# xdsopl/dwt

Hardware: AMD Instinct MI355X
Metric: Mpixels/s lossless encode+decode round-trip (higher is better)
Workload: dtype int32; 1 GPU; 4096x4096x1 8-bit synthetic smooth+noise frames, lossless, 128 frames per GPU per step (BASELINE.json configs[1] geometry); frames_per_gpu=128, parallelism=1 GPU

## Files before the change

dwt_amd/csrc/pack.hip:

```cpp
#include "hilbert_dev.h"

#include <stdlib.h>
#include <string.h>

namespace {

constexpr int TILE = 1024;
constexpr int NCUM = 32;
constexpr int MAX_PLANES = 16;
constexpr int MAX_SEGS = 3 * 16 * MAX_PLANES;
constexpr int SUB = 64;
constexpr int CHUNK = SUB * 64;
constexpr int GROUP = 64;

constexpr unsigned T_RUN = 0x0fffu, T_ESC = 0x0fffu, T_BREAK = 1u << 13, T_VOID = 1u << 14, T_NOSIGN = 1u << 15;

struct PackGeom {
	int levels, C, W, H;
	long total;
	const int *pyr;
	const short *fine16;
	unsigned lv16;
	unsigned sq_levels;
	int pixels[DWTX_MAX_LEVELS + 1];
// ... 1713 lines not shown

__global__ __launch_bounds__(1024) void k_chain_image(Work w)
{
	const int img = blockIdx.x;
	if (!w.slow[img])
		return;
	const ImgInfo &I = w.info[img];
	const long nchunks = ((long)I.T + CHUNK - 1) / CHUNK;
	const long ngroups = (nchunks + GROUP - 1) / GROUP;
	unsigned char *gentry = w.group_entry + img * w.NGS;
	if (threadIdx.x == 0) {
		int o = I.order0;
		for (long gq = 0; gq < ngroups; ++gq) {
			gentry[gq] = (unsigned char)o;
			o = w.glut[(img * w.NGS + gq) * 32 + o];
		}
	}
	__syncthreads();
	__threadfence_block();
	const unsigned char *lut = w.lut + img * w.NCS * 32;
	unsigned char *centry = w.chunk_entry + img * w.NCS;
	for (long gq = threadIdx.x; gq < ngroups; gq += 1024) {
		int o = gentry[gq];
		for (long c = gq * GROUP; c < min((gq + 1) * GROUP, nchunks); ++c) {
			centry[c] = (unsigned char)o;
			o = lut[c * 32 + o];
		}
	}
}

__device__ __forceinline__ void gorder_exact_body(const Work &w, unsigned *rows, long chunk, int img)
{
	const int lane = threadIdx.x & 63;
	const ImgInfo &I = w.info[img];
	const long T = I.T;
	const long nchunks = (T + CHUNK - 1) / CHUNK;
	if (chunk >= nchunks)
		return;
	const unsigned short *tok16 = w.tok16 + img * w.TS;
	const unsigned *big = w.tok_big + img * w.TS;
	wave_sync();
	stage_tokens(rows, tok16, chunk * CHUNK, T, lane);
	wave_sync();
	const long S = chunk * 64 + lane;
	const int o = w.sublut[((img * w.NCS + chunk) * 64 + lane) * 32 + w.chunk_entry[img * w.NCS + chunk]];
	const bool produces = S * SUB < T;
	unsigned tokbits = 0;
	unsigned long long rawbits = 0;
	walk_bits(rows + lane * WROW, big, S * SUB, o, 16, produces, w.brk_tok + (long)img * MAX_SEGS, w.seg_refs + (long)img * MAX_SEGS, I.K,
		tokbits, rawbits);
	unsigned long long total;
	const unsigned long long pre = wave_excl_scan64(produces ? tokbits + rawbits : 0ull, total);
	if (produces) {
		w.lane_bits[img * w.NCS * 64 + S] = pre;
		w.grp_ord[img * w.NCS * 64 + S] = (unsigned char)o;
	}
	if (lane == 0)
		w.chunk_bits[img * w.NCS + chunk] = total;
}

__global__ __launch_bounds__(256) void k_gorder_exact(Work w)
{
	__shared__ WalkLds lds[4];
	const int img = blockIdx.y;
	if (!w.slow[img])
		return;
	const long nvb = (w.NCS + 3) / 4;
	for (long vb = blockIdx.x; vb < nvb; vb += gridDim.x)
		gorder_exact_body(w, lds[threadIdx.x >> 6].tok, vb * 4 + (threadIdx.x >> 6), img);
}

constexpr int EWIN = 768;

struct EmitLds {
	unsigned tok[64 * HROW];
	unsigned win[EWIN];
};

__global__ __launch_bounds__(256) __attribute__((amdgpu_waves_per_eu(5))) void k_emit(Work w, unsigned *out, long out_words)
{
	__shared__ EmitLds lds[4];
	const int lane = threadIdx.x & 63, wv = threadIdx.x >> 6;
	const long wave = (long)blockIdx.x * 4 + wv;
	const int img = blockIdx.y;
	const ImgInfo &I = w.info[img];
	const long T = I.T;
	const long ngroups = (T + SUB - 1) / SUB;
	if (wave * 64 >= ngroups)
		return;
	const unsigned short *tok16 = w.tok16 + img * w.TS;
	const unsigned *big = w.tok_big + img * w.TS;
	const unsigned *srefs = w.seg_refs + (long)img * MAX_SEGS;
	const unsigned *btok = w.brk_tok + (long)img * MAX_SEGS;
	unsigned *rows = lds[wv].tok, *win = lds[wv].win;
	for (int i = lane; i < EWIN; i += 64)
		win[i] = 0u;
	const long S = wave * 64 + lane;
	const bool live = S < ngroups;
	const int per = w.slow[img] ? 64 : FSUBS;
	unsigned long long pos = 0;
	int o = 0;
	if (live) {
		pos = w.chunk_base[img * w.NCS + S / per] + w.lane_bits[img * w.NCS * 64 + S];
		o = w.grp_ord[img * w.NCS * 64 + S];
	}
	const long wbase = (long)(__shfl(pos, 0) >> 5);
	unsigned *dst = out + img * out_words;
	wave_sync();
	auto put_word = [&](long wi, unsigned v) {
		if (!v)
			return;
		const unsigned long rel = (unsigned long)(wi - wbase);
		if (rel < (unsigned long)EWIN)
			__hip_atomic_fetch_or((__attribute__((address_space(3))) unsigned *)win + rel, v, __ATOMIC_RELAXED, __HIP_MEMORY_SCOPE_WORKGROUP);
		else if (wi < out_words)
			atomicOr(dst + wi, v);
	};
	long widx = (long)(pos >> 5);
	int fill = (int)(pos & 31);
	unsigned long long acc = 0;
	auto append = [&](unsigned c, int n) {
		acc |= (unsigned long long)c << fill;
		fill += n;
		if (fill >= 32) {
			put_word(widx, (unsigned)acc);
			++widx;
			acc >>= 32;
			fill -= 32;
		}
	};
	const unsigned *my = rows + lane * HROW;
	const long tb = S * SUB;
	auto slow_token = [&](unsigned tk, long t) {
		if (!(tk & T_VOID)) {
			const unsigned v = token_run(tk, big, t);
			const int top = vli_top(o, v);
			const int z = top - o;
			const unsigned rem = v + (1u << o) - (1u << top);
			unsigned long long code = (1ull << z) | ((unsigned long long)rem << (z + 1));
			int len = z + 1 + top;
			if (!(tk & T_NOSIGN)) {
				code |= (unsigned long long)((tk >> 12) & 1u) << len;
				++len;
			}
			o = vli_next(top);
			append((unsigned)code, len < 32 ? len : 32);
			if (len > 32)
				append((unsigned)(code >> 32), len - 32);
		}
		if (tk & T_BREAK) {
			put_word(widx, (unsigned)acc);
			acc = 0;
			const long k = find_break_seg(btok, I.K, (unsigned)t);
			const unsigned long long at = ((unsigned long long)widx << 5) + (unsigned)fill;
			w.seg_rawoff[(long)img * MAX_SEGS + k] = at;
			const unsigned long long next = at + srefs[k];
			widx = (long)(next >> 5);
			fill = (int)(next & 31);
		}
	};
	auto code16 = [&](unsigned tk, unsigned &code, int &len) {
		const unsigned s = (tk & T_RUN) + (1u << o);
		const int top = 31 - __builtin_clz(s);
		const int z = top - o;
		const unsigned rem = s & bfm_mask((unsigned)top);
		const int l = z + 1 + top;
		code = (rem << (z + 1)) | (1u << z) | (((tk >> 12) & 1u) << l);
		len = l + ((tk & T_NOSIGN) ? 0 : 1);
		o = (int)__builtin_elementwise_sub_sat((unsigned)top, 2u);
	};
	HalfTokens staged = load_tokens_half(tok16, wave * CHUNK, T, lane, 0);
	for (int half = 0; half < 2; ++half) {
		if (half)
			wave_sync();
		deposit_tokens_half(rows, staged, lane);
		if (!half)
			staged = load_tokens_half(tok16, wave * CHUNK, T, lane, 1);
		wave_sync();
		if (!live)
			continue;
#pragma unroll 2
		for (int q8 = 0; q8 < 8; ++q8) {
			const int q = half * 8 + q8;
			const uint2 x2 = *reinterpret_cast<const uint2 *>(my + 2 * q8);
			const unsigned xs[2] = { x2.x, x2.y };
#pragma unroll
			for (int h = 0; h < 2; ++h) {
				const unsigned x = xs[h];
				if ((x & ((0x0f80u | T_BREAK | T_VOID) * 0x00010001u)) != 0u || o > 7) {
					slow_token(x & 0xffffu, tb + 4 * q + 2 * h);
					slow_token(x >> 16, tb + 4 * q + 2 * h + 1);
				} else {
					unsigned c0, c1;
					int l0, l1;
					code16(x & 0xffffu, c0, l0);
					code16(x >> 16, c1, l1);
					acc |= (unsigned long long)(c0 | (c1 << l0)) << fill;
					fill += l0 + l1;
					if (fill >= 32) {
						put_word(widx, (unsigned)acc);
						++widx;
						acc >>= 32;
						fill -= 32;
					}
				}
			}
		}
	}
	if (live)
		put_word(widx, (unsigned)acc);
	const long nlive = ngroups - wave * 64 < 64 ? ngroups - wave * 64 : 64;
	const long endw = __shfl(widx, (int)nlive - 1);
	wave_sync();
	for (int i = lane; i < EWIN; i += 64) {
		const long wi = wbase + i;
		if (wi - i + (i & ~63) > endw)
			break;
		if (wi > endw || wi >= out_words)
			continue;
		const unsigned v = win[i];
		if (wi > wbase && wi < endw)
			dst[wi] = v;
		else if (v)
			atomicOr(dst + wi, v);
	}
}

__global__ __launch_bounds__(1024) void k_bitscan(Work w, long capacity)
{
	__shared__ unsigned long long wsum[16];
	__shared__ unsigned long long carry;
	const int img = blockIdx.x;
	ImgInfo &I = w.info[img];
	const long nsub = ((long)I.T + SUB - 1) / SUB;
	const long nchunks = w.slow[img] ? ((long)I.T + CHUNK - 1) / CHUNK : (nsub + FSUBS - 1) / FSUBS;
	const unsigned long long *cb = w.chunk_bits + img * w.NCS;
	unsigned long long *base = w.chunk_base + img * w.NCS;
	const int lane = threadIdx.x & 63, wv = threadIdx.x >> 6;
	if (threadIdx.x == 0)
		carry = I.hdr_bits;
	__syncthreads();
	for (long b0 = 0; b0 < nchunks; b0 += 1024) {
		const long i = b0 + threadIdx.x;
		const unsigned long long v = i < nchunks ? cb[i] : 0ull;
		unsigned long long inc = v;
		for (int o = 1; o < 64; o <<= 1) {
			const unsigned long long t = __shfl_up(inc, o);
			if (lane >= o)
				inc += t;
		}
		if (lane == 63)
			wsum[wv] = inc;
		__syncthreads();
		unsigned long long woff = 0, all = 0;
		for (int k = 0; k < 16; ++k) {
			const unsigned long long s = wsum[k];
			woff += k < wv ? s : 0ull;
			all += s;
		}
		const unsigned long long c = carry;
		if (i < nchunks)
			base[i] = c + woff + inc - v;
		__syncthreads();
		if (threadIdx.x == 0)
			carry = c + all;
		__syncthreads();
	}
	if (threadIdx.x == 0) {
		const unsigned long long bits = carry;
		w.stream_bits[img] = bits;
		unsigned long long bytes = (bits + 7) >> 3;
		I.total_bits = bits;
		if (capacity > 0 && bytes > (unsigned long long)capacity) {
			bytes = (unsigned long long)capacity;
			if (bits >= 8ull * ((unsigned long long)capacity + 1))
				I.total_bits = bytes * 8;
		}
		I.nbytes = bytes;
		I.pad = w.slow[img];
	}
}

__global__ __launch_bounds__(256) void k_clear_stream(Work w, unsigned *out, long out_words)
{
	const int img = blockIdx.y;
	const long first = ((long)w.info[img].hdr_bits + 31) >> 5;
	long last = (long)((w.stream_bits[img] + 31) >> 5) + 4;
	last = last < out_words ? last : out_words;
	unsigned *base = out + img * out_words;
	const bool vec = ((uintptr_t)base & 15) == 0;
	for (long i = ((first & ~3l) >> 2) + (long)blockIdx.x * blockDim.x + threadIdx.x; i * 4 < last; i += (long)gridDim.x * blockDim.x) {
		unsigned *dst = base + i * 4;
		if (vec && i * 4 >= first && i * 4 + 4 <= last) {
			*reinterpret_cast<uint4 *>(dst) = make_uint4(0u, 0u, 0u, 0u);
		} else {
			for (int k = 0; k < 4; ++k)
				if (i * 4 + k >= first && i * 4 + k < last)
					dst[k] = 0u;
		}
	}
}

constexpr int REF_WIN = 2048;

__global__ __launch_bounds__(256) void k_refcopy(Work w, unsigned *out, long out_words)
{
	const int img = blockIdx.y;
	const int K = w.info[img].K;
	const int *eb = w.seg_ebase + (long)img * (MAX_SEGS + 1);
	const unsigned *refscum = w.ent_refscum + img * (w.ES + 1), *refw = w.ent_refw + img * (w.ES + 1);
	const unsigned short *erefs = w.ent_refs + img * w.ES;
	const unsigned *stage = w.stage + img * w.SW;
	unsigned *dst = out + img * out_words;
	__shared__ unsigned win[REF_WIN + 2];
	__shared__ unsigned wfirst[MAX_SEGS + 1];
	__shared__ unsigned wsum[4];
	{
		unsigned mine[3], sum = 0;
#pragma unroll
		for (int u = 0; u < 3; ++u) {
			const int k = 3 * (int)threadIdx.x + u;
			unsigned nwin = 0;
			if (k < K) {
				const unsigned n = w.seg_refs[(long)img * MAX_SEGS + k];
				if (n) {
					const unsigned long long D = w.seg_rawoff[(long)img * MAX_SEGS + k];
					const unsigned long words = (unsigned long)(((D + n - 1) >> 5) - (D >> 5) + 1);
					nwin = (unsigned)((words + REF_WIN - 1) / REF_WIN);
				}
			}
			mine[u] = nwin;
			sum += nwin;
		}
		unsigned total;
		const unsigned pre = block_excl_scan(sum, wsum, total);
		unsigned run = pre;
#pragma unroll
		for (int u = 0; u < 3; ++u) {
			const int k = 3 * (int)threadIdx.x + u;
			wfirst[k] = run;
			run += mine[u];
		}
		if (threadIdx.x == blockDim.x - 1)
			wfirst[MAX_SEGS] = run;
		__syncthreads();
	}
	const unsigned nwin_all = wfirst[K < MAX_SEGS ? K : MAX_SEGS];
	for (unsigned vw = blockIdx.x; vw < nwin_all; vw += gridDim.x) {
		int lo = 0, hi = K - 1;
		while (lo < hi) {
			const int mid = (lo + hi + 1) >> 1;
			if (wfirst[mid] <= vw)
				lo = mid;
			else
				hi = mid - 1;
		}
		const int k = lo;
		const unsigned wi = vw - wfirst[k];
		const unsigned n = w.seg_refs[(long)img * MAX_SEGS + k];
		const unsigned long long D = w.seg_rawoff[(long)img * MAX_SEGS + k];
		const long d0 = (long)(D >> 5), dl = (long)((D + n - 1) >> 5);
		const long ws = d0 + (long)wi * REF_WIN;
		const int nwords = (int)(dl - ws + 1 < REF_WIN ? dl - ws + 1 : REF_WIN);
		const long long x0 = ((long long)ws << 5) - (long long)D, x1 = x0 + 32ll * nwords;
		for (int i = threadIdx.x; i < nwords + 2; i += blockDim.x)
			win[i] = 0u;
		__syncthreads();
		const int e0 = eb[k], e1 = eb[k + 1];
		const unsigned cbase = refscum[e0];
		int a = e0, b = e1 - 1;
		while (a < b) {
			const int mid = (a + b + 1) >> 1;
			if ((long long)(refscum[mid] - cbase) <= (x0 > 0 ? x0 : 0))
				a = mid;
			else
				b = mid - 1;
		}
		for (int ea = a; ea < e1; ea += blockDim.x) {
			const int e = ea + (int)threadIdx.x;
			const long long c = e < e1 ? (long long)(refscum[e] - cbase) : x1;
			if (__syncthreads_and(c >= x1))
				break;
			const unsigned r = e < e1 ? erefs[e] : 0u;
			if (!r || c >= x1)
				continue;
			const unsigned *src = stage + refw[e];
			const int nsrc = (int)((r + 31u) >> 5);
			for (int jw = 0; jw < nsrc; ++jw) {
				const long long o = c + 32ll * jw - x0;
				if (o <= -32 || o >= 32ll * nwords)
					continue;
				const unsigned v = src[jw];
				const long long ob = o + 32;
				const int idx = (int)(ob >> 5), sh = (int)(ob & 31);
				if (v) {
					atomicOr(&win[idx], v << sh);
					if (sh && idx + 1 < nwords + 2)
						atomicOr(&win[idx + 1], v >> (32 - sh));
				}
			}
		}
		__syncthreads();
		for (int i = threadIdx.x; i < nwords; i += blockDim.x) {
			const long wd = ws + i;
			if (wd >= out_words)
				continue;
			const unsigned v = win[1 + i];
			if (wd == d0 || wd == dl) {
				if (v)
					atomicOr(dst + wd, v);
			} else {
				dst[wd] = v;
			}
		}
		__syncthreads();
	}
}

constexpr int IDX_THREADS = 832;
static_assert(IDX_THREADS > MAX_SEGS && IDX_THREADS % 64 == 0, "one lane per segment and one for the header");

__global__ __launch_bounds__(IDX_THREADS) void k_index(PackGeom g, Work w, dwtx_index *index)
{
	__shared__ unsigned long long wsum[IDX_THREADS / 64];
	__shared__ unsigned nxt[IDX_THREADS];
	__shared__ unsigned btok[MAX_SEGS], srefs[MAX_SEGS];
	const int img = blockIdx.x;
	const ImgInfo &I = w.info[img];
	dwtx_index &X = index[img];
	const int K = I.K;
	const bool whole = I.nbytes >= (w.stream_bits[img] + 7) >> 3;
	if (K <= 0 || I.pmax <= 0 || I.error || I.cut || !whole) {
		if (threadIdx.x == 0) {
			X.magic = DWTX_INDEX_MAGIC;
			X.W = g.W;
			X.H = g.H;
			X.C = g.C;
			X.nsegs = 0;
			X.reserved = 0;
			X.stream_bits = 0ull;
		}
		return;
	}
	const int k = threadIdx.x, lane = threadIdx.x & 63, wv = wave_in_block();
	const int *sd = w.seg_desc + (long)img * MAX_SEGS;
	int num = 0;
	if (k < K) {
		int c, l, p;
		seg_unpack(sd[k], c, l, p);
		num = g.pixels[l + 1] - g.pixels[l];
	}
	const long T = I.T;
	const unsigned short *tok16 = w.tok16 + img * w.TS;
	const unsigned *big = w.tok_big + img * w.TS;
	if (k < K) {
		btok[k] = w.brk_tok[(long)img * MAX_SEGS + k];
		srefs[k] = w.seg_refs[(long)img * MAX_SEGS + k];
	}
	long t0 = T - 1;
	if (k < K) {
		t0 = w.ent_tokbase[img * (w.ES + 1) + w.seg_ebase[(long)img * (MAX_SEGS + 1) + k]];
		nxt[k] = (tok16[t0] & T_VOID) ? (unsigned)(T - 1) : (unsigned)t0;
	} else {
		nxt[k] = (unsigned)(T - 1);
	}
	unsigned long long wtot;
	unsigned long long sym_base = wave_excl_scan64(((unsigned long long)num + 31ull) & ~31ull, wtot);
	if (lane == 0)
		wsum[wv] = wtot;
	__syncthreads();
	for (int i = 0; i < wv; ++i)
		sym_base += wsum[i];
	for (int d = 1; d < IDX_THREADS; d <<= 1) {
		const unsigned a = nxt[k], b = k + d < IDX_THREADS ? nxt[k + d] : a;
		__syncthreads();
		nxt[k] = a < b ? a : b;
		__syncthreads();
	}
	if (k > K)
		return;
	const unsigned j = k < K ? w.seg_run[(long)img * MAX_SEGS + k] : 0u;
	const long tt = j ? (long)nxt[k] : t0;
	const long S = tt / SUB;
	const int per = w.slow[img] ? 64 : FSUBS;
	unsigned long long pos = w.chunk_base[img * w.NCS + S / per] + w.lane_bits[img * w.NCS * 64 + S];
	int o = w.grp_ord[img * w.NCS * 64 + S];
	uint4 grp[8];
#pragma unroll
	for (int q = 0; q < 8; ++q)
		grp[q] = *reinterpret_cast<const uint4 *>(tok16 + S * SUB + 8 * q);
	const int before = (int)(tt - S * SUB);
	int kb = (int)find_break_seg(btok, K, (unsigned)(S * SUB));
#pragma unroll
	for (int q = 0; q < 32; ++q) {
		const uint4 x4 = grp[q >> 2];
		const unsigned x = (q & 3) == 0 ? x4.x : (q & 3) == 1 ? x4.y : (q & 3) == 2 ? x4.z : x4.w;
#pragma unroll
		for (int h = 0; h < 2; ++h) {
			const unsigned tk = h ? x >> 16 : x & 0xffffu;
			const long t = S * SUB + 2 * q + h;
			if (2 * q + h < before) {
				if (!(tk & T_VOID)) {
					const int top = vli_top(o, token_run(tk, big, t));
					pos += (unsigned)(2 * top - o + 1) + ((tk & T_NOSIGN) ? 0u : 1u);
					o = vli_next(top);
				}
				if (tk & T_BREAK)
					pos += srefs[kb++];
			}
		}
	}
	const unsigned v = token_run(tok16[tt], big, tt);
	if (k < K ? j != 0u : v != 0u) {
		const int top = vli_top(o, v);
		pos += (unsigned)(2 * top - o + 1);
		o = vli_next(top);
	}
	if (k < K) {
		dwtx_seg_index &e = X.seg[k];
		e.bit = pos;
		e.sym_base = sym_base;
		e.n1 = (unsigned)num - srefs[k];
		e.cnt = j ? v - j + 1u : 0u;
		e.desc = (unsigned)sd[k];
		e.order = (unsigned)o;
	} else {
		X.magic = DWTX_INDEX_MAGIC;
		X.W = g.W;
		X.H = g.H;
		X.C = g.C;
		X.nsegs = K;
		X.reserved = 0;
		X.stream_bits = pos;
	}
}

}


extern "C" int dwtx_encode_planes(dwtx_ctx *ctx, const int32_t *lin, int W, int H, int C, int n, long capacity,
	uint8_t *out, size_t out_stride, dwtx_stream_info *dev_info)
{
	return dwtx_encode_planes_ex(ctx, lin, nullptr, 0u, 0u, W, H, C, n, capacity, out, out_stride, dev_info, dwtx_p16{ nullptr, 0u },
		ctx ? ctx->enc_index : nullptr);
}

static int pack_geometry(dwtx_ctx *ctx, int W, int H, int C, int n, PackGeom &g, Work &w, dwtx_tiles &tiles)
{
	const int rc = dwtx_fill_geom(ctx, W, H, C, g, tiles);
	if (rc)
		return rc;
	g.tile_cnt = tiles.cnt;
	memset(&w, 0, sizeof(w));
	w.NT = tiles.NT;
	w.NTP = (tiles.NT + 3) / 4 * 4;
	const size_t nplanes = (size_t)n * C;
	const bool ok = carve(ctx, SLOT_PK_CUM, [&](Carve &c) {
		c.take(w.cum, nplanes * w.NT * NCUM);
		c.take(w.tile_mx, nplanes * w.NTP);
	});
	return ok ? DWTX_OK : DWTX_ERR_NOMEM;
}

int dwtx_hist_begin(dwtx_ctx *ctx, int W, int H, int C, int n, dwtx_hist_sink *sink)
{
	if (!ctx || !sink || (C != 1 && C != 3) || n < 1 || !dwtx_count_ok((long)n * C, DWTX_MAX_PLANES_PER_CALL, "planes"))
		return DWTX_ERR_ARG;
	DWTX_ENTER(ctx);
	DWTX_CHECK_DIMS(W, H);
	PackGeom g;
	Work w;
	dwtx_tiles tiles;
	const int rc = pack_geometry(ctx, W, H, C, n, g, w, tiles);
	if (rc)
		return rc;
	hipLaunchKernelGGL(k_hist_init, dim3(dwtx_cdiv(w.NT * (NCUM / 2), 256), n * C), dim3(256), 0, ctx->stream, g, w);
	DWTX_LAUNCH_CHECK();
	sink->cum32 = reinterpret_cast<unsigned *>(w.cum);
	sink->tile_mx = w.tile_mx;
	sink->NT = w.NT;
	sink->NTP = w.NTP;
	sink->tiles = tiles;
	return DWTX_OK;
}

#ifdef DWTX_DEBUG_HOOKS
extern "C" int dwtx_debug_hist_copy(dwtx_ctx *ctx, int W, int H, int C, int n, unsigned *host_cum32, unsigned *host_mx, int *NT, int *NTP, int *tile_first)
{
	PackGeom g;
	Work w;
	dwtx_tiles tiles;
	const int rc = pack_geometry(ctx, W, H, C, n, g, w, tiles);
	if (rc)
		return rc;
	*NT = w.NT;
	*NTP = w.NTP;
	for (int l = 0; l <= g.levels; ++l)
		tile_first[l] = tiles.tile_first[l];
	if (host_cum32) {
		DWTX_HIP(hipMemcpyAsync(host_cum32, w.cum, sizeof(unsigned) * 16 * (size_t)n * C * w.NT, hipMemcpyDeviceToHost, ctx->stream));
		DWTX_HIP(hipMemcpyAsync(host_mx, w.tile_mx, sizeof(unsigned) * (size_t)n * C * w.NTP, hipMemcpyDeviceToHost, ctx->stream));
		DWTX_HIP(hipStreamSynchronize(ctx->stream));
	}
	return DWTX_OK;
}
#endif

int dwtx_encode_planes_ex(dwtx_ctx *ctx, const int32_t *lin, const int32_t *pyr, unsigned sq_levels, unsigned hist_levels, int W, int H, int C,
	int n, long capacity, uint8_t *out, size_t out_stride, dwtx_stream_info *dev_info, dwtx_p16 p16, dwtx_index *dev_index)
{
	if (!ctx || !lin || !out || !dev_info || (C != 1 && C != 3) || n < 1 || (out_stride & 3) || out_stride < 8 ||
		!dwtx_count_ok((long)n * C, DWTX_MAX_PLANES_PER_CALL, "planes"))
		return DWTX_ERR_ARG;
	DWTX_ENTER(ctx);
	DWTX_CHECK_DIMS(W, H);
	if (sq_levels && (!pyr || (sq_levels & ~dwtx_square_levels(W, H)) || ((uintptr_t)pyr & 15)))
		return DWTX_ERR_ARG;
	PackGeom g;
	Work w;
	dwtx_tiles tiles;
	{
		const int rc = pack_geometry(ctx, W, H, C, n, g, w, tiles);
		if (rc)
			return rc;
	}
	g.pyr = pyr;
	g.sq_levels = sq_levels;
	g.fine16 = p16.planes;
	g.lv16 = p16.planes ? p16.levels : 0u;
	if (p16.planes && ((p16.levels & ~sq_levels) || ((uintptr_t)p16.planes & 15)))
		return DWTX_ERR_ARG;
	const int NT = tiles.NT;
	int hist_tiles = NT;
	for (int l = g.levels - 1; l >= 0 && ((hist_levels >> l) & 1u); --l)
		hist_tiles = tiles.tile_first[l];
	w.ES = (long)NT * C * MAX_PLANES + 16;
	w.TS = ((long)C * (g.total - g.pixels[0]) + MAX_SEGS + 8 + 63) / 64 * 64;
	w.NCS = (w.TS / SUB + FSUBS - 1) / FSUBS + 2;
	w.NGS = (w.NCS + GROUP - 1) / GROUP;
	w.NCB = (w.ES + CARRY_BLOCK - 1) / CARRY_BLOCK;
	w.SW = (long)(((unsigned long long)C * (unsigned long long)(g.total - g.pixels[0]) * (MAX_PLANES - 1) + 31) / 32) + w.ES + 64;
	const int nplanes = n * C;

	const size_t imgs = n;
	char *small = carve(ctx, SLOT_PK_SMALL, [&](Carve &c) {
		c.take(w.info, imgs);
		c.take(w.slow, imgs);
		c.take(w.stream_bits, imgs);
		c.take(w.seg_desc, imgs * MAX_SEGS);
		c.take(w.seg_ebase, imgs * (MAX_SEGS + 1));
		c.take(w.seg_refs, imgs * MAX_SEGS);
		c.take(w.seg_rawoff, imgs * MAX_SEGS);
		c.take(w.brk_tok, imgs * MAX_SEGS);
		c.take(w.segidx, imgs * 48 * MAX_PLANES);
		c.take(w.live, imgs * 48);
		c.take(w.seg_run, imgs * MAX_SEGS);
	});
	if (!small)
		return DWTX_ERR_NOMEM;
	DWTX_HIP(hipMemsetAsync(w.info, 0, (char *)w.seg_desc - (char *)w.info, ctx->stream));
	if (ctx->opt[DWTX_OPT_EXACT_ORDERS])
		DWTX_HIP(hipMemsetD32Async((hipDeviceptr_t)w.slow, 1, (size_t)n, ctx->stream));

	char *ent = carve(ctx, SLOT_PK_ENT, [&](Carve &c) {
		c.take(w.ent_ones, imgs * w.ES);
		c.take(w.ent_zeros, imgs * w.ES);
		c.take(w.ent_refs, imgs * w.ES);
		c.take(w.ent_tz, imgs * w.ES);
		c.take(w.ent_seg, imgs * w.ES);
		c.take(w.ent_tokbase, imgs * (w.ES + 1));
		c.take(w.ent_refscum, imgs * (w.ES + 1));
		c.take(w.ent_refw, imgs * (w.ES + 1));
		c.take(w.carry_agg, imgs * w.NCB);
		c.take(w.carry_in, imgs * w.NCB);
		c.take(w.ent_blk, imgs * w.NCB * 3);
	});
	if (!ent)
		return DWTX_ERR_NOMEM;

	w.tok_big = (unsigned *)dwtx_scratch(ctx, SLOT_PK_TOKBIG, sizeof(unsigned) * (size_t)n * w.TS);
	w.tok16 = (unsigned short *)dwtx_scratch(ctx, SLOT_PK_TOK16, sizeof(unsigned short) * (size_t)n * w.TS);
	w.stage = (unsigned *)dwtx_scratch(ctx, SLOT_PK_STAGE, sizeof(unsigned) * (size_t)n * w.SW);
	if (!w.tok_big || !w.tok16 || !w.stage)
		return DWTX_ERR_NOMEM;

	w.sublut = (unsigned char *)dwtx_scratch(ctx, SLOT_PK_LUT, (size_t)n * w.NCS * 64 * 32);
	char *ch = carve(ctx, SLOT_PK_CHUNK, [&](Carve &c) {
		c.take(w.lut, imgs * w.NCS * 32);
		c.take(w.glut, imgs * w.NGS * 32);
		c.take(w.chunk_entry, imgs * w.NCS);
		c.take(w.group_entry, imgs * w.NGS);
		c.take(w.grp_ord, imgs * w.NCS * 64);
		c.take(w.chunk_bits, imgs * w.NCS);
		c.take(w.chunk_base, imgs * w.NCS);
		c.take(w.lane_bits, imgs * w.NCS * 64);
	});
	if (!w.sublut || !ch)
		return DWTX_ERR_NOMEM;

	hipStream_t s = ctx->stream;
	const long out_words = (long)(out_stride / 4);
	unsigned *outw = (unsigned *)out;

	if (hist_tiles > 0)
		hipLaunchKernelGGL(k_hist, dim3(dwtx_cdiv(hist_tiles, 4 * HIST_TPW), nplanes), dim3(256), 0, s, g, lin, w, hist_levels);
	hipLaunchKernelGGL(k_plan, dim3(n), dim3(1024), 0, s, g, lin, w, outw, out_words, capacity);
	hipLaunchKernelGGL(k_entries_count, dim3((unsigned)w.NCB, n), dim3(ENT_BLOCK), 0, s, g, w);
	hipLaunchKernelGGL(k_entries_blocks, dim3(n), dim3(ENT_BLOCK), 0, s, w);
	hipLaunchKernelGGL(k_entries_finish, dim3((unsigned)w.NCB, n), dim3(ENT_BLOCK), 0, s, w);
	hipLaunchKernelGGL(k_entries_segs, dim3(n), dim3(ENT_BLOCK), 0, s, w);
	hipLaunchKernelGGL(k_cut, dim3(n), dim3(ENT_BLOCK), 0, s, w, capacity, (int)(ctx->opt[DWTX_OPT_NO_CAPACITY_CUT] != 0));
	hipLaunchKernelGGL(k_code<false>, dim3(dwtx_cdiv(NT, 4), C, n), dim3(256), 0, s, g, lin, w);
	hipLaunchKernelGGL(k_code<true>, dim3(dwtx_cdiv(NT, 4) < 64 ? dwtx_cdiv(NT, 4) : 64, C, n), dim3(256), 0, s, g, lin, w);
	hipLaunchKernelGGL(k_carry_local, dim3((unsigned)w.NCB, n), dim3(CARRY_THREADS), 0, s, w);
	hipLaunchKernelGGL(k_carry_blocks, dim3(n), dim3(CARRY_BLOCK), 0, s, w);
// ... 24 lines not shown
```

Before: 99110 Mpixels/s.

## Restructure refcopy to distribute source words across threads with shared bitmap rank lookup

Rewrites the reference-copy kernel so that, rather than each thread serially walking all source words of one entry, a round of up to 256 entries is staged into a shared bitmap. All threads then cooperatively scan the contiguous staged source words, mapping each word back to its entry by popcount rank. The window-to-segment lookup now comes from per-thread registers instead of a shared binary search. The entry-start search becomes a block-wide count-based narrowing, and the output writeback uses aligned 128-bit stores. This is meant to remove load imbalance and serial per-entry loops. The cost is extra shared memory, more barriers per round, and more complex indexing.

```diff
diff --git a/dwt_amd/csrc/pack.hip b/dwt_amd/csrc/pack.hip
--- a/dwt_amd/csrc/pack.hip
+++ b/dwt_amd/csrc/pack.hip
@@ -2039,115 +2039,187 @@
 }
 
 constexpr int REF_WIN = 2048;
-
-__global__ __launch_bounds__(256) void k_refcopy(Work w, unsigned *out, long out_words)
-{
-	const int img = blockIdx.y;
-	const int K = w.info[img].K;
+constexpr int REF_ENTS = 256;
+constexpr int REF_SRC = REF_WIN + 2 * REF_ENTS;
+static_assert(TILE <= 1024 && REF_WIN + 3 * (TILE / 32) + REF_ENTS <= REF_SRC, "a round's staging words fit the bitmap");
+
+struct RefWin {
+	int e0, e1;
+	unsigned wi, n;
+	unsigned long long D;
+};
+
+__global__ __launch_bounds__(REF_ENTS) void k_refcopy(Work w, unsigned *out, long out_words)
+{
+	const int img = blockIdx.y, tid = threadIdx.x, lane = tid & 63, wv = tid >> 6;
 	const int *eb = w.seg_ebase + (long)img * (MAX_SEGS + 1);
 	const unsigned *refscum = w.ent_refscum + img * (w.ES + 1), *refw = w.ent_refw + img * (w.ES + 1);
 	const unsigned short *erefs = w.ent_refs + img * w.ES;
 	const unsigned *stage = w.stage + img * w.SW;
 	unsigned *dst = out + img * out_words;
 	__shared__ unsigned win[REF_WIN + 2];
-	__shared__ unsigned wfirst[MAX_SEGS + 1];
-	__shared__ unsigned wsum[4];
+	__shared__ unsigned bm[REF_SRC / 32];
+	__shared__ unsigned short grp[REF_SRC / 32 + 1];
+	__shared__ int entoff[REF_ENTS + 32];
+	__shared__ unsigned wsum[4], wcnt[4], wend[4];
+	__shared__ RefWin cur;
+	__shared__ int more;
+	static_assert(MAX_SEGS == 3 * REF_ENTS, "three segments per thread");
+	unsigned mine[3], nref[3], pre;
+	unsigned long long at[3];
+	int ebv[4];
+	unsigned nwin_all;
 	{
-		unsigned mine[3], sum = 0;
 #pragma unroll
 		for (int u = 0; u < 3; ++u) {
-			const int k = 3 * (int)threadIdx.x + u;
+			nref[u] = w.seg_refs[(long)img * MAX_SEGS + 3 * tid + u];
+			at[u] = w.seg_rawoff[(long)img * MAX_SEGS + 3 * tid + u];
+		}
+#pragma unroll
+		for (int u = 0; u < 4; ++u)
+			ebv[u] = eb[3 * tid + u];
+		const int K = w.info[img].K;
+		unsigned sum = 0;
+#pragma unroll
+		for (int u = 0; u < 3; ++u) {
 			unsigned nwin = 0;
-			if (k < K) {
-				const unsigned n = w.seg_refs[(long)img * MAX_SEGS + k];
-				if (n) {
-					const unsigned long long D = w.seg_rawoff[(long)img * MAX_SEGS + k];
-					const unsigned long words = (unsigned long)(((D + n - 1) >> 5) - (D >> 5) + 1);
-					nwin = (unsigned)((words + REF_WIN - 1) / REF_WIN);
-				}
+			if (3 * tid + u < K && nref[u]) {
+				const unsigned long long D = at[u];
+				const unsigned long words = (unsigned long)(((D + nref[u] - 1) >> 5) - (D >> 5) + 1);
+				nwin = (unsigned)((words + REF_WIN - 1) / REF_WIN);
 			}
 			mine[u] = nwin;
 			sum += nwin;
 		}
-		unsigned total;
-		const unsigned pre = block_excl_scan(sum, wsum, total);
-		unsigned run = pre;
-#pragma unroll
-		for (int u = 0; u < 3; ++u) {
-			const int k = 3 * (int)threadIdx.x + u;
-			wfirst[k] = run;
-			run += mine[u];
-		}
-		if (threadIdx.x == blockDim.x - 1)
-			wfirst[MAX_SEGS] = run;
+		pre = block_excl_scan(sum, wsum, nwin_all);
+	}
+	for (unsigned vw = blockIdx.x; vw < nwin_all; vw += gridDim.x) {
+		{
+			unsigned run = pre;
+#pragma unroll
+			for (int u = 0; u < 3; ++u) {
+				if (vw - run < mine[u]) {
+					cur.e0 = ebv[u];
+					cur.e1 = ebv[u + 1];
+					cur.wi = vw - run;
+					cur.n = nref[u];
+					cur.D = at[u];
+				}
+				run += mine[u];
+			}
+		}
+		for (int i = tid; i < REF_WIN + 2; i += REF_ENTS)
+			win[i] = 0u;
 		__syncthreads();
-	}
-	const unsigned nwin_all = wfirst[K < MAX_SEGS ? K : MAX_SEGS];
-	for (unsigned vw = blockIdx.x; vw < nwin_all; vw += gridDim.x) {
-		int lo = 0, hi = K - 1;
-		while (lo < hi) {
-			const int mid = (lo + hi + 1) >> 1;
-			if (wfirst[mid] <= vw)
-				lo = mid;
-			else
-				hi = mid - 1;
-		}
-		const int k = lo;
-		const unsigned wi = vw - wfirst[k];
-		const unsigned n = w.seg_refs[(long)img * MAX_SEGS + k];
-		const unsigned long long D = w.seg_rawoff[(long)img * MAX_SEGS + k];
+		const int e0 = cur.e0, e1 = cur.e1;
+		const unsigned wi = cur.wi, n = cur.n;
+		const unsigned long long D = cur.D;
 		const long d0 = (long)(D >> 5), dl = (long)((D + n - 1) >> 5);
 		const long ws = d0 + (long)wi * REF_WIN;
+		if (ws >= out_words) {
+			__syncthreads();
+			continue;
+		}
 		const int nwords = (int)(dl - ws + 1 < REF_WIN ? dl - ws + 1 : REF_WIN);
 		const long long x0 = ((long long)ws << 5) - (long long)D, x1 = x0 + 32ll * nwords;
-		for (int i = threadIdx.x; i < nwords + 2; i += blockDim.x)
-			win[i] = 0u;
-		__syncthreads();
-		const int e0 = eb[k], e1 = eb[k + 1];
 		const unsigned cbase = refscum[e0];
-		int a = e0, b = e1 - 1;
-		while (a < b) {
-			const int mid = (a + b + 1) >> 1;
-			if ((long long)(refscum[mid] - cbase) <= (x0 > 0 ? x0 : 0))
-				a = mid;
-			else
-				b = mid - 1;
-		}
-		for (int ea = a; ea < e1; ea += blockDim.x) {
-			const int e = ea + (int)threadIdx.x;
-			const long long c = e < e1 ? (long long)(refscum[e] - cbase) : x1;
-			if (__syncthreads_and(c >= x1))
+		int a = e0;
+		if (wi) {
+			int len = e1 - e0;
+			while (len > 1) {
+				const int step = (len + REF_ENTS - 1) / REF_ENTS;
+				const bool le = tid * step < len && (long long)(refscum[a + tid * step] - cbase) <= x0;
+				const int cnt = __syncthreads_count(le);
+				a += (cnt - 1) * step;
+				len -= (cnt - 1) * step;
+				len = len < step ? len : step;
+			}
+		}
+		for (int ea = a; ea < e1; ea += REF_ENTS) {
+			const int e = ea + tid;
+			const bool valid = e < e1;
+			const long long c = valid ? (long long)(refscum[e] - cbase) : x1;
+			const unsigned r = valid ? erefs[e] : 0u;
+			const unsigned gbase = refw[ea];
+			const unsigned s0 = valid ? refw[e] - gbase : 0u;
+			const unsigned nsrc = (r + 31u) >> 5;
+			const bool has = r != 0u && c < x1 && s0 + nsrc <= (unsigned)REF_SRC;
+			const unsigned long long bal = __ballot(has);
+			if (tid < REF_SRC / 32)
+				bm[tid] = 0u;
+			if (lane == 0)
+				wcnt[wv] = (unsigned)__popcll(bal);
+			if (has && !((bal >> lane) >> 1))
+				wend[wv] = s0 + nsrc;
+			if (tid == REF_ENTS - 1)
+				more = valid && c < x1;
+			__syncthreads();
+			unsigned rank = (unsigned)popc_below(bal), nsrc_all = 0;
+#pragma unroll
+			for (int k = 0; k < 4; ++k) {
+				const unsigned cnt = wcnt[k];
+				rank += k < wv ? cnt : 0u;
+				nsrc_all = cnt ? wend[k] : nsrc_all;
+			}
+			const bool again = more != 0;
+			if (has) {
+				entoff[rank] = (int)(c - x0) - 32 * (int)s0;
+				atomicOr(&bm[s0 >> 5], 1u << (s0 & 31u));
+				const unsigned g = (s0 + 31u) >> 5;
+				if (32u * g < s0 + nsrc)
+					grp[g] = (unsigned short)rank;
+			}
+			__syncthreads();
+			const unsigned *src = stage + gbase;
+			for (unsigned sb = tid; sb < nsrc_all; sb += 4 * REF_ENTS) {
+				unsigned v[4];
+#pragma unroll
+				for (int u = 0; u < 4; ++u) {
+					const unsigned s = sb + u * REF_ENTS;
+					v[u] = s < nsrc_all ? src[s] : 0u;
+				}
+#pragma unroll
+				for (int u = 0; u < 4; ++u) {
+					const unsigned s = sb + u * REF_ENTS;
+					if (!v[u])
+						continue;
+					const unsigned g = s >> 5;
+					const unsigned starts = bm[g] & ((2u << (s & 31u)) - 1u) & ~1u;
+					const unsigned rk = grp[g] + (unsigned)__popc(starts);
+					const long long o = (long long)entoff[rk < REF_ENTS + 31u ? rk : REF_ENTS + 31u] + 32ll * s;
+					if (o <= -32 || o >= 32ll * nwords)
+						continue;
+					const long long ob = o + 32;
+					const int idx = (int)(ob >> 5), sh = (int)(ob & 31);
+					atomicOr(&win[idx], v[u] << sh);
+					if (sh)
+						atomicOr(&win[idx + 1], v[u] >> (32 - sh));
+				}
+			}
+			__syncthreads();
+			if (!again)
 				break;
-			const unsigned r = e < e1 ? erefs[e] : 0u;
-			if (!r || c >= x1)
+		}
+		const int lead = (int)((4u - (unsigned)(((uintptr_t)(dst + ws) >> 2) & 3u)) & 3u);
+		for (int i0 = lead - 4 + 4 * tid; i0 < nwords; i0 += 4 * REF_ENTS) {
+			const long wd0 = ws + i0;
+			if (i0 >= 0 && i0 + 4 <= nwords && wd0 > d0 && wd0 + 3 < dl && wd0 + 4 <= out_words) {
+				*reinterpret_cast<uint4 *>(dst + wd0) = make_uint4(win[1 + i0], win[2 + i0], win[3 + i0], win[4 + i0]);
 				continue;
-			const unsigned *src = stage + refw[e];
-			const int nsrc = (int)((r + 31u) >> 5);
-			for (int jw = 0; jw < nsrc; ++jw) {
-				const long long o = c + 32ll * jw - x0;
-				if (o <= -32 || o >= 32ll * nwords)
+			}
+#pragma unroll
+			for (int j = 0; j < 4; ++j) {
+				const int i = i0 + j;
+				const long wd = ws + i;
+				if (i < 0 || i >= nwords || wd >= out_words)
 					continue;
-				const unsigned v = src[jw];
-				const long long ob = o + 32;
-				const int idx = (int)(ob >> 5), sh = (int)(ob & 31);
-				if (v) {
-					atomicOr(&win[idx], v << sh);
-					if (sh && idx + 1 < nwords + 2)
-						atomicOr(&win[idx + 1], v >> (32 - sh));
+				const unsigned v = win[1 + i];
+				if (wd == d0 || wd == dl) {
+					if (v)
+						atomicOr(dst + wd, v);
+				} else {
+					dst[wd] = v;
 				}
-			}
-		}
-		__syncthreads();
-		for (int i = threadIdx.x; i < nwords; i += blockDim.x) {
-			const long wd = ws + i;
-			if (wd >= out_words)
-				continue;
-			const unsigned v = win[1 + i];
-			if (wd == d0 || wd == dl) {
-				if (v)
-					atomicOr(dst + wd, v);
-			} else {
-				dst[wd] = v;
 			}
 		}
 		__syncthreads();
```

After: 99650 Mpixels/s (median of 6 runs). Within noise of the previous version (+0.5%).
